# dominikh/jello

Hardware: AMD Instinct MI355X
Metric: Mpixels/sec fine-raster + paths/sec, 100k-path 4096^2 scene (higher is better)
Workload: dtype f32

## Files before the change

jello_amd/csrc/kernels_flatten.hip:

```cpp
#include <hip/hip_runtime.h>
__shared__ double fl_atan_tab[9];
#define JD_ATAN_TAB_LDS fl_atan_tab
#include "kcommon.h"
#define FF_INLINE __device__ __forceinline__
#include "flatten_fast.h"

using namespace jk;
using namespace jd;

namespace {

struct CubicParams { float th0, th1, chord_len, err; };
struct EulerParams { float th0, th1, k0, k1, ch; };
struct CubicPoints { V2 p0, p1, p2, p3; };
struct PointDeriv { V2 point, deriv; };
struct PathTagData { uint32_t tag_byte; MonoidK<5> monoid; };

#define DERIV_THRESH 1e-6f
#define DERIV_THRESH_SQUARED (DERIV_THRESH * DERIV_THRESH)
#define DERIV_EPS 1e-6f
#define SUBDIV_LIMIT (1.0f / 65536.0f)
#define K1_THRESH 1e-3f
#define DIST_THRESH 1e-3f
#define TANGENT_THRESH 1e-6f
// ... 777 lines not shown
        bool is_stroke_cap_marker = (g.tag.tag_byte & JL_PATH_TAG_SUBPATH_END) != 0u;
        if (is_stroke_cap_marker) {
            V2 tangent = cubic_start_tangent(pts.p0, pts.p1, pts.p2, pts.p3);
            V2 offset_tangent = offset * normalize(tangent);
            V2 n = v2(offset_tangent.y * -1.0f, offset_tangent.x * 1.0f);
            draw_cap<EMIT>(o, path_ix, (style_flags & JL_STYLE_FLAGS_START_CAP_MASK) >> 2, pts.p0, pts.p0 - n, pts.p0 + n, -offset_tangent,
                           transform);
        } else {
            const float TT = TANGENT_THRESH * TANGENT_THRESH;
            V2 tan_prev = cubic_end_tangent(pts.p0, pts.p1, pts.p2, pts.p3);
            if (dot(tan_prev, tan_prev) < TT) tan_prev = v2(TANGENT_THRESH, 0.0f);
            V2 offset_tangent = offset * normalize(tan_prev);
            V2 n_prev = v2(offset_tangent.y * -1.0f, offset_tangent.x * 1.0f);
            if (sub < 2u) {
                V2 tan_start = cubic_start_tangent(pts.p0, pts.p1, pts.p2, pts.p3);
                if (dot(tan_start, tan_start) < TT) tan_start = v2(TANGENT_THRESH, 0.0f);
                V2 n_start = offset * normalize(v2(-tan_start.y, tan_start.x));
                job.valid = true; job.cubic = pts; job.local_to_device = transform;
                if (sub == 0u) { job.offset = offset; job.start_p = pts.p0 + n_start; job.end_p = pts.p3 + n_prev; }
                else { job.offset = -offset; job.start_p = pts.p0 - n_start; job.end_p = pts.p3 - n_prev; }
            } else {
                PathTagData ntag = compute_tag_monoid(s, ix + 1u);
                CubicPoints npts = read_path_segment(s, ntag, true);
                bool n_is_closed = (ntag.tag_byte & JL_PATH_TAG_SEG_TYPE) == JL_PATH_TAG_LINETO;
                bool n_is_marker = (ntag.tag_byte & JL_PATH_TAG_SUBPATH_END) != 0u;
                bool do_join = !n_is_marker || n_is_closed;
                if (do_join) {
                    V2 tan_next = cubic_start_tangent(npts.p0, npts.p1, npts.p2, npts.p3);
                    if (dot(tan_next, tan_next) < TT) tan_next = v2(TANGENT_THRESH, 0.0f);
                    V2 tnn = normalize(tan_next);
                    V2 n_next = v2((offset * tnn.y) * -1.0f, (offset * tnn.x) * 1.0f);
                    draw_join<EMIT>(o, path_ix, style_flags, pts.p3, tan_prev, tan_next, n_prev, n_next, transform);
                } else {
                    draw_cap<EMIT>(o, path_ix, (style_flags & JL_STYLE_FLAGS_END_CAP_MASK), pts.p3, pts.p3 + n_prev, pts.p3 - n_prev, offset_tangent,
                                   transform);
                }
            }
        }
    } else {
        job.valid = true; job.cubic = pts; job.local_to_device = transform;
        job.offset = 0.0f; job.start_p = pts.p0; job.end_p = pts.p3;
    }
}

#ifndef FLQ_STACK
#define FLQ_STACK 448u
#endif
#ifndef FLQ_LEAVES
#define FLQ_LEAVES 640u
#endif
#ifndef FLQ_MAX_LEVEL
#define FLQ_MAX_LEVEL 9u
#endif
struct FlBatch {
    uint32_t jhead[64];
    uint32_t stack[FLQ_STACK];
    uint32_t l_tpos[FLQ_LEAVES];
    uint16_t l_key[FLQ_LEAVES];
    uint16_t l_link[FLQ_LEAVES];
    uint32_t unsure[128];
    uint32_t n_stack, n_leaves, bail, n_unsure;
};
JD float lanef(float v, uint32_t src) { return u2f((uint32_t)__builtin_amdgcn_ds_bpermute((int)(src << 2), (int)f2u(v))); }
JD uint32_t laneu(uint32_t v, uint32_t src) { return (uint32_t)__builtin_amdgcn_ds_bpermute((int)(src << 2), (int)v); }

struct NodeResult {
    bool accept;
    CubicParams cp;
    V2 es_p0, es_p1;
    bool ends_at_one;
};
struct NodeEnds {
    V2 last_p, last_q;
    float last_t;
    V2 point, deriv;
    float t1;
};
JD NodeEnds node_ends(V2 p0, V2 p1, V2 p2, V2 p3, uint32_t level, uint32_t t0_u) {
    const float dt = u2f((127u - level) << 23);
    const float t0 = (float)t0_u * dt;
    NodeEnds r;
    if (t0_u == 0u) {
        r.last_p = p0;
        r.last_q = p1 - p0;
        if (dot(r.last_q, r.last_q) < DERIV_THRESH_SQUARED) r.last_q = eval_cubic_and_deriv(p0, p1, p2, p3, DERIV_EPS).deriv;
        r.last_t = 0.0f;
    } else {
        PointDeriv pq0 = eval_cubic_and_deriv(p0, p1, p2, p3, t0);
        r.last_t = t0;
        if (dot(pq0.deriv, pq0.deriv) < DERIV_THRESH_SQUARED) {
            PointDeriv n0 = eval_cubic_and_deriv(p0, p1, p2, p3, t0 - DERIV_EPS);
            pq0.deriv = n0.deriv;
            pq0.point = n0.point;
            r.last_t = t0 - DERIV_EPS;
        }
        r.last_p = pq0.point;
        r.last_q = pq0.deriv;
    }
    float t1 = t0 + dt;
    PointDeriv this_pq1 = eval_cubic_and_deriv(p0, p1, p2, p3, t1);
    if (dot(this_pq1.deriv, this_pq1.deriv) < DERIV_THRESH_SQUARED) {
        PointDeriv new_pq1 = eval_cubic_and_deriv(p0, p1, p2, p3, t1 - DERIV_EPS);
        this_pq1.deriv = new_pq1.deriv;
        if (t1 < 1.0f) {
            this_pq1.point = new_pq1.point;
            t1 = t1 - DERIV_EPS;
        }
    }
    r.point = this_pq1.point;
    r.deriv = this_pq1.deriv;
    r.t1 = t1;
    return r;
}
JD NodeResult node_test(V2 p0, V2 p1, V2 p2, V2 p3, float scale, uint32_t level, uint32_t t0_u) {
    const float tol = 0.25f;
    const float dt = u2f((127u - level) << 23);
    const NodeEnds ne = node_ends(p0, p1, p2, p3, level, t0_u);
    const float actual_dt = ne.t1 - ne.last_t;
    NodeResult r;
    r.cp = cubic_from_points_derivs(ne.last_p, ne.point, ne.last_q, ne.deriv, actual_dt);
    r.accept = r.cp.err * scale <= tol || dt <= SUBDIV_LIMIT;
    r.es_p0 = ne.last_p;
    r.es_p1 = ne.point;
    r.ends_at_one = ne.t1 == 1.0f;
    return r;
}
JD int node_test_fast(V2 p0, V2 p1, V2 p2, V2 p3, float scale, uint32_t level, uint32_t t0_u, float* v_est, float* delta) {
    const float tol = 0.25f;
    const NodeEnds ne = node_ends(p0, p1, p2, p3, level, t0_u);
    const float actual_dt = ne.t1 - ne.last_t;
    const V2 chord = ne.point - ne.last_p;
    const float chord_squared = dot(chord, chord);
    const V2 q0 = ne.last_q, q1 = ne.deriv;
    *v_est = 0.0f; *delta = 0.0f;
    if (chord_squared < DERIV_THRESH_SQUARED) {
        const float chord_err = sqrt_((float)(9.0 / 32.0) * (dot(q0, q0) + dot(q1, q1))) * actual_dt;
        return (chord_err * scale <= tol) ? ffast::FF_ACCEPT : ffast::FF_REJECT;
    }
    const float chord_len = FF_SQRT(chord_squared);
    const float sc = actual_dt * FF_RCP(chord_squared);
    const V2 h0 = v2(q0.x * chord.x + q0.y * chord.y, q0.y * chord.x - q0.x * chord.y);
    const V2 h1 = v2(q1.x * chord.x + q1.y * chord.y, q1.x * chord.y - q1.y * chord.x);
    const float len0 = FF_SQRT(h0.x * h0.x + h0.y * h0.y), len1 = FF_SQRT(h1.x * h1.x + h1.y * h1.y);
    return ffast::ff_decide(h0.x, h0.y, len0, h1.x, h1.y, len1, len0 * sc, len1 * sc, chord_len, scale, tol, v_est, delta);
}
JD CubicParams piece_angles(const NodeEnds& ne) {
    const V2 chord = ne.point - ne.last_p;
    const float chord_squared = dot(chord, chord);
    CubicParams r;
    r.err = 0.0f;
    if (chord_squared < DERIV_THRESH_SQUARED) {
        r.th0 = 0.0f; r.th1 = 0.0f; r.chord_len = DERIV_THRESH;
        return r;
    }
    const V2 q0 = ne.last_q, q1 = ne.deriv;
    const V2 h0 = v2(q0.x * chord.x + q0.y * chord.y, q0.y * chord.x - q0.x * chord.y);
    const V2 h1 = v2(q1.x * chord.x + q1.y * chord.y, q1.x * chord.y - q1.y * chord.x);
    r.th0 = atan2_(h0.y, h0.x);
    r.th1 = atan2_(h1.y, h1.x);
    r.chord_len = sqrt_(chord_squared);
    return r;
}

struct PieceParams {
    EulerParams ep;
    float n, noff, int0, integral;
    uint32_t n_u, robust;
};
JD PieceParams piece_params(const CubicParams& cp, float scale, float offset) {
    const float tol = 0.25f;
    PieceParams r;
    r.ep = es_params_from_angles(cp.th0, cp.th1);
    const EulerParams& ep = r.ep;
    float k0 = ep.k0 - 0.5f * ep.k1;
    float k1 = ep.k1;
    float normalized_offset = offset / cp.chord_len;
    float dist_scaled = normalized_offset * ep.ch;
    float scale_multiplier = sqrt_(0.125f * scale * cp.chord_len / (ep.ch * tol));
    float a = 0.0f, b = 0.0f, integral = 0.0f, int0 = 0.0f, n_frac;
    uint32_t robust = 0u;
    if (abs_(k1) < K1_THRESH) {
        float k = ep.k0;
        n_frac = sqrt_(abs_(k * (k * dist_scaled + 1.0f)));
        robust = 1u;
    } else if (abs_(dist_scaled) < DIST_THRESH) {
        a = k1;
        b = k0;
        int0 = pow_1_5_signed(b);
        float int1 = pow_1_5_signed(a + b);
        integral = int1 - int0;
        n_frac = (float)(2.0 / 3.0) * integral / a;
        robust = 2u;
    } else {
        a = -2.0f * dist_scaled * k1;
        b = -1.0f - 2.0f * dist_scaled * k0;
        int0 = espc_int_approx(b);
        float int1 = espc_int_approx(a + b);
        integral = int1 - int0;
        float k_peak = k0 - k1 * b / a;
        float integrand_peak = sqrt_(abs_(k_peak * (k_peak * dist_scaled + 1.0f)));
        n_frac = integral * integrand_peak / a;
    }
    r.n = clamp_(ceil_(n_frac * scale_multiplier), 1.0f, 100.0f);
    r.n_u = to_u32(r.n);
    r.noff = normalized_offset;
    r.int0 = int0;
    r.integral = integral;
    r.robust = robust;
    return r;
}

#ifdef FL_FAST_CHECK
__device__ uint32_t g_ff_stats[8];
#endif
#ifndef FL_WAVES_PER_EU
#define FL_WAVES_PER_EU 4
#endif
#ifndef FL_BLOCKS_PER_CU
#define FL_BLOCKS_PER_CU 4
#endif
#ifdef FL_TIMING
#define FL_TL_WAVES 8192u
#define FL_TL_BATCHES 15u
#define FL_TL_WORDS (2u + 3u * FL_TL_BATCHES)
__device__ unsigned long long g_fl_timeline[FL_TL_WAVES * FL_TL_WORDS];
#endif
__global__ __launch_bounds__(JL_WG) __attribute__((amdgpu_waves_per_eu(FL_WAVES_PER_EU, FL_WAVES_PER_EU))) void k_flatten_items(const JlConfig* __restrict__ cfg, Buf<uint32_t> scene, Buf<JlTagMonoid> tag_monoids,
                                                         Buf<JlPathBbox> path_bboxes, const uint32_t* __restrict__ list,
                                                         uint32_t* __restrict__ counters, uint32_t cap, uint32_t* __restrict__ counts,
                                                         FlTemp T, uint32_t debug) {
    __shared__ FlBatch sh_batch[JL_WG / 64];
    Scene s;
    s.cfg = cfg; s.scene = scene; s.tag_monoids = tag_monoids;
    uint32_t n_heavy = umin_(counters[0], cap), n_light = umin_(counters[FL_CTR_LIGHT], cap - n_heavy);
    uint32_t n = n_heavy + n_light;
    const uint32_t units_h = n_heavy / 64u + (n_heavy % 64u != 0u ? 1u : 0u);
    const uint32_t units = units_h + n_light / 64u + (n_light % 64u != 0u ? 1u : 0u);
    const uint32_t n_groups = umin_(umax_(gridDim.x / FL_BLOCKS_PER_CU, 1u), FL_DEAL_GROUPS), group = blockIdx.x % n_groups;
    if (group >= units) return;
#ifdef FL_TIMING
    const unsigned long long tl_entry = wall_clock64();
    const uint32_t tl_wave = blockIdx.x * (JL_WG / 64u) + (threadIdx.x >> 6);
    uint32_t tl_n = 0u;
#endif
    atan_tab_fill();
    __syncthreads();
    const uint32_t lane = lane_id();
    FlBatch& B = sh_batch[threadIdx.x >> 6];
    Out<true> o;
    o.cfg = cfg; o.T = T; o.home_s = o.home_r = blockIdx.x % T.K; o.failed_s = o.failed_r = false; o.slot = 0u;
    if ((debug & 1u) != 0u) o.home_s = o.home_r = 0u;
#ifdef FL_SOAK_HOME0
    o.home_s = o.home_r = 0u;
#endif
    o.cursor = 0u; o.a_first = 0u; o.a_spos = 0u; o.a_rpos = 0u;
    for (;;) {
        uint32_t k = 0u;
        if (lane == 0u) k = atomicAdd(&counters[FL_CTR_DEAL + FL_DEAL_STRIDE * group], 1u);
        k = (uint32_t)__builtin_amdgcn_readfirstlane((int)k);
        const uint32_t u = k * n_groups + group;
        if (u >= units) break;
        const bool heavy = u < units_h;
        const uint32_t t_first = heavy ? u * 64u : n_heavy + (u - units_h) * 64u;
        const uint32_t t_end = umin_(t_first + 64u, heavy ? n_heavy : n);
        const uint32_t t = t_first + lane;
#ifdef FL_TIMING
        const unsigned long long tl_start = wall_clock64() | (heavy ? 1ull << 63 : 0ull);
        uint32_t tl_info = 0u;
#define FL_TL_END()                                                                                      \
    do {                                                                                                 \
        if (lane == 0u && tl_wave < FL_TL_WAVES && tl_n < FL_TL_BATCHES) {                               \
            g_fl_timeline[tl_wave * FL_TL_WORDS + 2u + 3u * tl_n] = tl_start;                            \
            g_fl_timeline[tl_wave * FL_TL_WORDS + 3u + 3u * tl_n] = wall_clock64();                      \
            g_fl_timeline[tl_wave * FL_TL_WORDS + 4u + 3u * tl_n] = tl_info;                             \
        }                                                                                                \
        tl_n++;                                                                                          \
    } while (0)
#else
#define FL_TL_END() do {} while (0)
#endif
        if (__builtin_amdgcn_ballot_w64(o.failed_s) != 0ull) { o.home_s = fl_next_home(T, o.home_s, 0); o.failed_s = false; }
        if (__builtin_amdgcn_ballot_w64(o.failed_r) != 0ull) { o.home_r = fl_next_home(T, o.home_r, 1); o.failed_r = false; }
        EulerJob job;
        job.valid = false; job.path_ix = 0u; job.trans_ix = 0u; job.offset = 0.0f;
        job.start_p = v2(0, 0); job.end_p = v2(0, 0);
        job.cubic.p0 = job.cubic.p1 = job.cubic.p2 = job.cubic.p3 = v2(0, 0);
        job.local_to_device = xf_identity();
        uint32_t slot = FL_INVALID;
        if (t < t_end) {
            slot = heavy ? list[t] : list[cap - 1u - (t - n_heavy)];
            o.slot = slot; o.cursor = 0u; o.a_first = 0u; o.a_spos = 0u; o.a_rpos = 0u;
            uint32_t path_ix;
            run_item<true>(cfg, s, o, slot, job, path_ix);
            if (!job.valid) counts[slot] = o.cursor;
        }
        EulerLane e;
        euler_begin(e, job);
        const bool active = job.valid && !e.done;
        if (__builtin_amdgcn_ballot_w64(active) == 0ull) {
            FL_TL_END();
            continue;
        }
        B.jhead[lane] = 0u;
        {
            const uint64_t am = __builtin_amdgcn_ballot_w64(active);
            if (active) B.stack[(uint32_t)__builtin_popcountll(am & ((1ull << lane) - 1ull))] = lane;
            if (lane == 0u) { B.n_stack = (uint32_t)__builtin_popcountll(am); B.n_leaves = 0u; B.bail = 0u; B.n_unsure = 0u; }
        }
        wave_fence();
#ifdef FL_SPLIT_NO_A
        if (lane == 0u) B.n_stack = 0u;
        wave_fence();
#endif
        for (;;) {
#ifdef FL_TIMING
            tl_info += 1u << 16;
#endif
            const uint32_t ns = (uint32_t)__builtin_amdgcn_readfirstlane((int)B.n_stack);
            const uint32_t nu = (uint32_t)__builtin_amdgcn_readfirstlane((int)B.n_unsure);
            if (ns == 0u && nu == 0u) break;
            const bool exact_round = ns == 0u || nu >= 64u;
            const uint32_t take = umin_(exact_round ? nu : ns, 64u);
            const bool has = lane < take;
            const uint32_t node = has ? (exact_round ? B.unsure[nu - 1u - lane] : B.stack[ns - 1u - lane]) : 0u;
            wave_fence();
            const uint32_t j = node & 63u, level = (node >> 6) & 31u, t0_u = node >> 11;
            const V2 jp0 = v2(lanef(e.p0.x, j), lanef(e.p0.y, j)), jp1 = v2(lanef(e.p1.x, j), lanef(e.p1.y, j));
            const V2 jp2 = v2(lanef(e.p2.x, j), lanef(e.p2.y, j)), jp3 = v2(lanef(e.p3.x, j), lanef(e.p3.y, j));
            const float scale = lanef(e.scale, j);
            int kind = ffast::FF_UNSURE;
            if (exact_round) {
                if (has) kind = node_test(jp0, jp1, jp2, jp3, scale, level, t0_u).accept ? ffast::FF_ACCEPT : ffast::FF_REJECT;
            } else if (has) {
                float v_est, delta;
                kind = node_test_fast(jp0, jp1, jp2, jp3, scale, level, t0_u, &v_est, &delta);
#ifdef FL_FAST_CHECK
            }
            if (!exact_round) {
                bool c_unsure = false, c_contra = false, c_viol = false;
                if (has) {
                    float v2_, d2_;
                    const int k2 = node_test_fast(jp0, jp1, jp2, jp3, scale, level, t0_u, &v2_, &d2_);
                    const NodeResult rx = node_test(jp0, jp1, jp2, jp3, scale, level, t0_u);
                    const float vx = rx.cp.err * scale;
                    c_unsure = k2 == ffast::FF_UNSURE;
                    c_contra = (k2 == ffast::FF_ACCEPT && !rx.accept) || (k2 == ffast::FF_REJECT && rx.accept);
                    c_viol = (d2_ > 0.0f && !(abs_(v2_ - vx) <= d2_)) || (d2_ == 0.0f && k2 != ffast::FF_UNSURE && v2_ != 0.0f);
                }
                const uint32_t n0 = (uint32_t)__builtin_popcountll(__builtin_amdgcn_ballot_w64(has));
                const uint32_t n1 = (uint32_t)__builtin_popcountll(__builtin_amdgcn_ballot_w64(c_unsure));
                const uint32_t n2 = (uint32_t)__builtin_popcountll(__builtin_amdgcn_ballot_w64(c_contra));
                const uint32_t n3 = (uint32_t)__builtin_popcountll(__builtin_amdgcn_ballot_w64(c_viol));
                if (lane == 0u) {
                    atomicAdd(&g_ff_stats[0], n0);
                    if (n1) atomicAdd(&g_ff_stats[1], n1);
                    if (n2) atomicAdd(&g_ff_stats[2], n2);
                    if (n3) atomicAdd(&g_ff_stats[3], n3);
                }
#endif
            }
            const bool acc = has && kind == ffast::FF_ACCEPT, rej = has && kind == ffast::FF_REJECT, uns = has && kind == ffast::FF_UNSURE;
            const uint64_t accm = __builtin_amdgcn_ballot_w64(acc), rejm = __builtin_amdgcn_ballot_w64(rej), unsm = __builtin_amdgcn_ballot_w64(uns);
            const uint32_t n_acc = (uint32_t)__builtin_popcountll(accm), n_rej = (uint32_t)__builtin_popcountll(rejm);
            const uint32_t n_uns = (uint32_t)__builtin_popcountll(unsm);
            const uint32_t nl = (uint32_t)__builtin_amdgcn_readfirstlane((int)B.n_leaves);
            const uint32_t ns_left = exact_round ? ns : ns - take, nu_left = exact_round ? nu - take : nu;
            const bool too_deep = __builtin_amdgcn_ballot_w64(rej && level + 1u > FLQ_MAX_LEVEL) != 0ull;
            if (too_deep || ns_left + 2u * n_rej > FLQ_STACK || nl + n_acc > FLQ_LEAVES) {
                if (lane == 0u) B.bail = 1u;
                wave_fence();
                break;
            }
            const uint64_t below = (1ull << lane) - 1ull;
            if (rej) {
                const uint32_t pos = ns_left + 2u * (uint32_t)__builtin_popcountll(rejm & below);
                B.stack[pos] = j | ((level + 1u) << 6) | ((2u * t0_u + 1u) << 11);
                B.stack[pos + 1u] = j | ((level + 1u) << 6) | ((2u * t0_u) << 11);
            }
            if (acc) {
                const uint32_t li = nl + (uint32_t)__builtin_popcountll(accm & below);
                B.l_tpos[li] = node;
                B.l_key[li] = (uint16_t)((t0_u << (FLQ_MAX_LEVEL - level)) << 7);
                const uint32_t prev = atomicExch(&B.jhead[j], li + 1u);
                B.l_link[li] = (uint16_t)((j << 10) | prev);
            }
            if (uns) B.unsure[nu_left + (uint32_t)__builtin_popcountll(unsm & below)] = node;
            if (lane == 0u) { B.n_stack = ns_left + 2u * n_rej; B.n_leaves = nl + n_acc; B.n_unsure = nu_left + n_uns; }
            wave_fence();
        }
        const bool bail = (uint32_t)__builtin_amdgcn_readfirstlane((int)B.bail) != 0u;
        const uint32_t nl = bail ? 0u : (uint32_t)__builtin_amdgcn_readfirstlane((int)B.n_leaves);
#ifdef FL_TIMING
        tl_info = (tl_info & 0x7fff0000u) | (nl & 0xffffu) | (bail ? 1u << 31 : 0u);
#endif
        uint32_t rec_base = 0u;
        if (nl != 0u && lane == 0u) rec_base = fl_grab<1>(T, o.home_r, nl, o.failed_r);
        rec_base = (uint32_t)__builtin_amdgcn_readlane((int)rec_base, 0);
#ifdef FL_SPLIT_NO_B
        for (uint32_t lbase = nl; lbase < nl; lbase += 64u) {
#else
        for (uint32_t lbase = 0u; lbase < nl; lbase += 64u) {
#endif
            const uint32_t li = lbase + lane;
            const bool has = li < nl;
            const uint32_t node = has ? B.l_tpos[li] : 0u;
            const uint32_t j = node & 63u, level = (node >> 6) & 31u, t0_u = node >> 11;
            const V2 jp0 = v2(lanef(e.p0.x, j), lanef(e.p0.y, j)), jp1 = v2(lanef(e.p1.x, j), lanef(e.p1.y, j));
            const V2 jp2 = v2(lanef(e.p2.x, j), lanef(e.p2.y, j)), jp3 = v2(lanef(e.p3.x, j), lanef(e.p3.y, j));
            const float scale = lanef(e.scale, j), offset = lanef(e.offset, j);
            const uint32_t j_slot = laneu(slot, j), j_path = laneu(e.path_ix, j), j_trans = laneu(e.trans_ix, j);
            const float j_tsx = lanef(e.t_start.x, j), j_tsy = lanef(e.t_start.y, j), j_tex = lanef(e.t_end.x, j), j_tey = lanef(e.t_end.y, j);
            if (has) {
                const NodeEnds ne = node_ends(jp0, jp1, jp2, jp3, level, t0_u);
                const CubicParams cp = piece_angles(ne);
                const PieceParams pp = piece_params(cp, scale, offset);
                const uint32_t fl = pp.robust | ((ne.t1 == 1.0f) ? 4u : 0u) | ((offset >= 0.0f) ? 8u : 0u) | ((offset == 0.0f) ? 16u : 0u) |
                                    ((t0_u == 0u) ? 32u : 0u);
                const uint32_t r = rec_base + li;
                if (rec_base != FL_INVALID)
                    piece_record_write(T.recs + (size_t)r * 4u, ne.last_p, ne.point, pp.ep.th0, pp.ep.th1, pp.int0, pp.integral, pp.noff, j_slot, j_path,
                                       j_trans, fl, 0u, v2(j_tsx, j_tsy), v2(j_tex, j_tey));
                B.l_key[li] = (uint16_t)(B.l_key[li] | pp.n_u);
            }
        }
        wave_fence();
        if (nl != 0u) {
            uint32_t total = 0u;
            if (active)
                for (uint32_t q = B.jhead[lane]; q != 0u; q = B.l_link[q - 1u] & 1023u) total += B.l_key[q - 1u] & 127u;
            if (active) counts[slot] = total;
            const uint32_t incl = wave_incl_scan_u32(total);
            const uint32_t batch_total = (uint32_t)__builtin_amdgcn_readlane((int)incl, 63);
            const bool together = batch_total <= ((debug & 4u) != 0u ? 48u : FL_MAX_GRAB);
            uint32_t grab = 0u;
            if (together) {
                if (lane == 0u) grab = fl_grab<0>(T, o.home_s, batch_total, o.failed_s);
            } else if (active && total != 0u) {
                grab = fl_grab<0>(T, o.home_s, total, o.failed_s);
            }
            for (uint32_t li = lane; li < nl; li += 64u) {
                const uint32_t j = B.l_link[li] >> 10, key = B.l_key[li];
                uint32_t first = 0u;
                for (uint32_t q = B.jhead[j]; q != 0u; q = B.l_link[q - 1u] & 1023u) {
                    const uint32_t k2 = B.l_key[q - 1u];
                    if ((k2 >> 7) < (key >> 7)) first += k2 & 127u;
                }
                B.l_tpos[li] = first;
            }
            {
                const uint32_t base0 = (uint32_t)__builtin_amdgcn_readlane((int)grab, 0);
                B.unsure[lane] = together ? (base0 == FL_INVALID ? FL_INVALID : base0 + (incl - total)) : grab;
            }
            wave_fence();
            for (uint32_t li = lane; li < nl; li += 64u) {
                const uint32_t j = B.l_link[li] >> 10, key = B.l_key[li], first = B.l_tpos[li];
                const uint32_t r = rec_base + li, jb = B.unsure[j];
                if (rec_base != FL_INVALID && (key >> 7) != 0u) ((uint32_t*)T.recs)[(size_t)r * 16u + 12u] = first;
                if (jb == FL_INVALID) continue;
                if (rec_base != FL_INVALID) piece_slots_write(T.sinfo, jb + first, key & 127u, r);
                else for (uint32_t i = 0u; i < (key & 127u); i++) T.sinfo[jb + first + i] = make_uint2(0u, 0u);
            }
            wave_fence();
        }
        if (__builtin_expect(bail, 0)) {
            o.slot = slot; o.cursor = 0u; o.a_first = 0u; o.a_spos = 0u; o.a_rpos = 0u;
            bool have = active;
            auto finish = [&]() -> bool {
                if (e.done && have) {
                    counts[o.slot] = o.cursor;
                    have = false;
                }
                return __builtin_amdgcn_ballot_w64(!e.done) != 0ull;
            };
            flatten_euler_wave(o, e, finish);
        }
        FL_TL_END();
    }
#ifdef FL_TIMING
    if (lane == 0u && tl_wave < FL_TL_WAVES) {
        g_fl_timeline[tl_wave * FL_TL_WORDS] = tl_entry;
        g_fl_timeline[tl_wave * FL_TL_WORDS + 1u] = tl_n;
    }
#endif
#undef FL_TL_END
}

#ifndef FL_LINES_WAVES_PER_EU
#define FL_LINES_WAVES_PER_EU 4
#endif
__global__ __launch_bounds__(JL_WG) __attribute__((amdgpu_waves_per_eu(FL_LINES_WAVES_PER_EU, FL_LINES_WAVES_PER_EU))) void k_flatten_lines(const JlConfig* __restrict__ cfg, Buf<uint32_t> scene, const uint32_t* __restrict__ counters,
                                                         FlTemp T, const uint32_t* __restrict__ bases, uint32_t n_slots, Buf<JlLineSoup> lines) {
    atan_tab_fill();
    const uint32_t lines_lim = umin_(cfg->lines_size, lines.n);
    const uint2* __restrict__ sinfo = T.sinfo;
    const uint4* __restrict__ recs = T.recs;
    const uint32_t n_r = T.K * T.R;
    uint32_t ru[FL_MAX_REGIONS], used[FL_MAX_REGIONS];
    uint32_t units = 0u;
#pragma unroll
    for (uint32_t c = 0u; c < FL_MAX_REGIONS; c++) {
        ru[c] = units;
        used[c] = c < T.K ? umin_(counters[FL_CTR_CURSOR + FL_CUR_STRIDE * c], T.R) : 0u;
        units += (used[c] + JL_WG - 1u) / JL_WG;
    }
    auto fetch_info = [&](uint32_t u) -> uint2 {
        if (u >= units) return make_uint2(0u, 0u);
        uint32_t c = 0u, first_unit = 0u, in_use = used[0];
#pragma unroll
        for (uint32_t q = 1u; q < FL_MAX_REGIONS; q++)
            if (u >= ru[q] && used[q] != 0u) { c = q; first_unit = ru[q]; in_use = used[q]; }
        const uint32_t in_region = (u - first_unit) * JL_WG + threadIdx.x;
        return in_region < in_use ? sinfo[(size_t)c * T.R + in_region] : make_uint2(0u, 0u);
    };
    auto state_of = [&](uint2 si) -> uint32_t {
        if (si.x >= n_r) return 0u;
        return (si.y & FL_INFO_PIECE) != 0u ? 2u : ((si.y & FL_INFO_DIRECT) != 0u ? 1u : 0u);
    };
    auto fetch_rec = [&](uint32_t state, uint32_t r, uint4& r0, uint4& r1, uint4& r2, uint4& r3) {
        r0 = r1 = r2 = r3 = make_uint4(0u, 0u, 0u, 0u);
        const uint4* rec = recs + (size_t)r * 4u;
        if (state != 0u) { r0 = rec[0]; r1 = rec[1]; }
        if (state == 2u) { r2 = rec[2]; r3 = rec[3]; }
    };
    const uint32_t G = gridDim.x;
    uint2 si_a = fetch_info(blockIdx.x), si_b = fetch_info(blockIdx.x + G);
    uint32_t st_a = state_of(si_a);
    uint4 a0, a1, a2, a3;
    fetch_rec(st_a, si_a.x, a0, a1, a2, a3);
    for (uint32_t u = blockIdx.x; u < units; u += G) {
        const uint32_t st = st_a;
        const uint2 si = si_a;
        const uint4 r0 = a0, r1 = a1, r2 = a2, r3 = a3;
        si_a = si_b;
        st_a = state_of(si_a);
        fetch_rec(st_a, si_a.x, a0, a1, a2, a3);
        si_b = fetch_info(u + 2u * G);
        uint32_t widx[3] = {0xffffffffu, 0xffffffffu, 0xffffffffu};
        uint2 wdat[3] = {make_uint2(0u, 0u), make_uint2(0u, 0u), make_uint2(0u, 0u)};
        if (st == 1u) {
            const uint32_t item = r0.x, k = r0.y;
            if (item < n_slots) {
                const uint32_t dst = bases[item] + k;
                if (dst < lines_lim) {
                    widx[0] = dst * 3u; wdat[0] = make_uint2(r0.z, 0u);
                    widx[1] = dst * 3u + 1u; wdat[1] = make_uint2(r1.x, r1.y);
                    widx[2] = dst * 3u + 2u; wdat[2] = make_uint2(r1.z, r1.w);
                }
            }
        } else if (st == 2u) {
            const uint32_t n_u = (si.y >> 8) & 127u, i = si.y & 127u;
            const uint32_t flags = r2.w & 63u;
            const bool last_of_item = i + 1u == n_u && (flags & 4u) != 0u;
            const uint32_t slot = r2.y, k = ((flags & 32u) != 0u ? 0u : r3.x) + i;
            Xf tr;
            if ((flags & 16u) != 0u) {
                tr = xf_identity();
            } else {
                uint32_t tb = cfg->layout.transform_base + (r2.w >> 6) * 6u;
                tr.m0 = u2f(scene.rd(tb)); tr.m1 = u2f(scene.rd(tb + 1u)); tr.m2 = u2f(scene.rd(tb + 2u));
                tr.m3 = u2f(scene.rd(tb + 3u)); tr.t0 = u2f(scene.rd(tb + 4u)); tr.t1 = u2f(scene.rd(tb + 5u));
            }
            const uint32_t slot_base = slot < n_slots ? bases[slot] : 0u;
            V2 lp1;
            if (last_of_item) {
                lp1 = v2(u2f(r3.z), u2f(r3.w));
#if defined(FL_LSPLIT) && FL_LSPLIT == 1
            } else if (true) {
                lp1 = v2(u2f(r0.x) + (float)i, u2f(r0.w) + u2f(r1.x) + u2f(r1.y) + u2f(r1.z) + u2f(r1.w) + u2f(r2.x));
#endif
            } else {
                const EulerParams ep = es_params_from_angles(u2f(r1.x), u2f(r1.y));
                const float noff = u2f(r2.x), n = (float)n_u;
                const float tt = (float)(i + 1u) / n;
                float sarg = tt;
                const uint32_t robust = flags & 3u;
                if (robust != 1u) {
                    const float k0 = ep.k0 - 0.5f * ep.k1, k1 = ep.k1;
                    const float dist_scaled = noff * ep.ch;
                    const float int0 = u2f(r1.z), integral = u2f(r1.w);
                    float a, b;
                    if (robust == 2u) {
                        a = k1;
                        b = k0;
                    } else {
                        a = -2.0f * dist_scaled * k1;
                        b = -1.0f - 2.0f * dist_scaled * k0;
                    }
                    float uu = integral * tt + int0;
                    float inv;
                    if (robust == 2u) inv = pow23_abs_(uu) * sign_(uu); else inv = espc_int_inv_approx(uu);
                    sarg = (inv - b) / a;
                }
                lp1 = es_seg_eval_with_offset(v2(u2f(r0.x), u2f(r0.y)), v2(u2f(r0.z), u2f(r0.w)), ep, sarg, noff);
            }
            const V2 q = xf_apply(tr, lp1);
            if (slot < n_slots) {
                const uint32_t dst = slot_base + k;
                const bool fwd = (flags & 8u) != 0u;
                const bool has_next = !last_of_item && dst + 1u < lines_lim;
                const uint2 hdr = make_uint2(r2.z, 0u), pt = make_uint2(f2u(q.x), f2u(q.y));
                if (dst < lines_lim) {
                    if (k == 0u) {
                        uint2* w = (uint2*)lines.p;
                        const V2 qs = xf_apply(tr, v2(u2f(r3.x), u2f(r3.y)));
                        w[(size_t)dst * 3u] = hdr;
                        w[(size_t)dst * 3u + (fwd ? 1u : 2u)] = make_uint2(f2u(qs.x), f2u(qs.y));
                    }
                    widx[0] = dst * 3u + (fwd ? 2u : 1u); wdat[0] = pt;
                    if (has_next) {
                        widx[1] = dst * 3u + 3u; wdat[1] = hdr;
                        widx[2] = dst * 3u + (fwd ? 4u : 5u); wdat[2] = pt;
                    }
                }
            }
        }
        {
            uint2* w = (uint2*)lines.p;
#pragma unroll
            for (int j = 0; j < 3; j++)
#if defined(FL_LSPLIT) && FL_LSPLIT == 2
                if (widx[j] == 0xfffffffeu) w[widx[j]] = wdat[j];
#else
                if (widx[j] != 0xffffffffu) w[widx[j]] = wdat[j];
#endif
        }
    }
}

JD uint32_t fkey(float f) { uint32_t b = f2u(f); return (b & 0x80000000u) ? ~b : (b | 0x80000000u); }
JD float fkey_inv(uint32_t k) { return u2f((k & 0x80000000u) ? (k & 0x7fffffffu) : ~k); }

JD bool fb_tag_has_extent(const uint32_t* __restrict__ bases, uint32_t n_tags, const JlLineSoup* lines, uint32_t total, uint32_t pos) {
    uint32_t g = 0u, ge = n_tags;
    while (ge - g > 1u) {
        const uint32_t mid = g + (ge - g) / 2u;
        if (umin_(bases[3u * mid], total) <= pos) g = mid; else ge = mid;
    }
    const uint32_t lo = umin_(bases[3u * g], total);
    const uint32_t hi = (g + 1u < n_tags) ? umin_(bases[3u * g + 3u], total) : total;
    float bx0 = 1e31f, by0 = 1e31f, bx1 = -1e31f, by1 = -1e31f;
    for (uint32_t i = lo; i < hi; i++) {
        const JlLineSoup l = lines[i];
        bx0 = fmin_(bx0, fmin_(l.p0[0], l.p1[0])); by0 = fmin_(by0, fmin_(l.p0[1], l.p1[1]));
        bx1 = fmax_(bx1, fmax_(l.p0[0], l.p1[0])); by1 = fmax_(by1, fmax_(l.p0[1], l.p1[1]));
    }
    return bx1 > bx0 || by1 > by0;
}

JD void fb_merge(Buf<JlPathBbox> path_bboxes, uint32_t path_ix, int32_t x0, int32_t y0, int32_t x1, int32_t y1, bool atomic) {
    if (!path_bboxes.ok(path_ix)) return;
    if (x0 == 0x7fffffff && y0 == 0x7fffffff && x1 == (int32_t)0x80000000 && y1 == (int32_t)0x80000000) return;
    JlPathBbox* out = &path_bboxes.p[path_ix];
    if (!atomic) {
        out->x0 = imin_(out->x0, x0); out->y0 = imin_(out->y0, y0);
        out->x1 = imax_(out->x1, x1); out->y1 = imax_(out->y1, y1);
    } else {
        const int32_t cx0 = __hip_atomic_load(&out->x0, __ATOMIC_RELAXED, __HIP_MEMORY_SCOPE_AGENT);
        const int32_t cy0 = __hip_atomic_load(&out->y0, __ATOMIC_RELAXED, __HIP_MEMORY_SCOPE_AGENT);
        const int32_t cx1 = __hip_atomic_load(&out->x1, __ATOMIC_RELAXED, __HIP_MEMORY_SCOPE_AGENT);
        const int32_t cy1 = __hip_atomic_load(&out->y1, __ATOMIC_RELAXED, __HIP_MEMORY_SCOPE_AGENT);
        if (x0 < cx0) atomicMin(&out->x0, x0);
        if (y0 < cy0) atomicMin(&out->y0, y0);
        if (x1 > cx1) atomicMax(&out->x1, x1);
        if (y1 > cy1) atomicMax(&out->y1, y1);
    }
}

#define FB_NONE 0xffffffffu
#ifndef FB_TARGET_WAVES
#define FB_TARGET_WAVES 2048u
#endif
__global__ __launch_bounds__(JL_WG) void k_flatten_bbox(const JlConfig* __restrict__ cfg, const JlBump* __restrict__ bump,
                                                        const uint32_t* __restrict__ bases, uint32_t n_slots, Buf<JlLineSoup> lines,
                                                        Buf<JlPathBbox> path_bboxes, uint32_t* __restrict__ zero, uint32_t zero_n) {
    for (uint32_t i = blockIdx.x * JL_WG + threadIdx.x; i < zero_n; i += gridDim.x * JL_WG) zero[i] = 0u;
    const uint32_t n_tags = n_slots / 3u;
    const uint32_t total = umin_(umin_(bump->lines, cfg->lines_size), lines.n);
    const uint32_t lane = lane_id();
    const uint32_t n_waves = (gridDim.x * JL_WG) >> 6;
    const uint32_t batches = umin_(umax_(((total + 63u) / 64u) / FB_TARGET_WAVES, 1u), 8u);
    for (uint64_t start64 = (uint64_t)((blockIdx.x * JL_WG + threadIdx.x) >> 6) * batches * 64u; start64 < total;
         start64 += (uint64_t)n_waves * batches * 64u) {
        const uint32_t start = (uint32_t)start64;
        const uint32_t end = (uint32_t)(start64 + (uint64_t)batches * 64u < total ? start64 + (uint64_t)batches * 64u : total);
        uint32_t p_before = FB_NONE;
        if (start > 0u) p_before = lines.p[start - 1u].path_ix;
        bool skip_before = false;
// ... 185 lines not shown
```

Measured before the change: 21430.

## Dedupe identical adjacent curves and speculatively evaluate child nodes in idle lanes

```diff
diff --git a/jello_amd/csrc/kernels_flatten.hip b/jello_amd/csrc/kernels_flatten.hip
--- a/jello_amd/csrc/kernels_flatten.hip
+++ b/jello_amd/csrc/kernels_flatten.hip
@@ -1103,10 +1103,19 @@
             continue;
         }
         B.jhead[lane] = 0u;
+        uint64_t followers;
         {
             const uint64_t am = __builtin_amdgcn_ballot_w64(active);
-            if (active) B.stack[(uint32_t)__builtin_popcountll(am & ((1ull << lane) - 1ull))] = lane;
-            if (lane == 0u) { B.n_stack = (uint32_t)__builtin_popcountll(am); B.n_leaves = 0u; B.bail = 0u; B.n_unsure = 0u; }
+#define FL_DIFF_BELOW(v) ((uint32_t)__builtin_amdgcn_update_dpp(0, (int)f2u(v), 0x138, 0xf, 0xf, false) ^ f2u(v))
+            const uint32_t diff = FL_DIFF_BELOW(e.p0.x) | FL_DIFF_BELOW(e.p0.y) | FL_DIFF_BELOW(e.p1.x) | FL_DIFF_BELOW(e.p1.y) | FL_DIFF_BELOW(e.p2.x) |
+                                  FL_DIFF_BELOW(e.p2.y) | FL_DIFF_BELOW(e.p3.x) | FL_DIFF_BELOW(e.p3.y) | FL_DIFF_BELOW(e.scale);
+#undef FL_DIFF_BELOW
+            const bool both = lane != 0u && ((am >> ((lane - 1u) & 63u)) & 3ull) == 3ull;
+            const bool follower = both && diff == 0u && (debug & 16u) == 0u;
+            followers = __builtin_amdgcn_ballot_w64(follower);
+            const uint64_t lead = am & ~followers;
+            if (active && !follower) B.stack[(uint32_t)__builtin_popcountll(lead & ((1ull << lane) - 1ull))] = lane;
+            if (lane == 0u) { B.n_stack = (uint32_t)__builtin_popcountll(lead); B.n_leaves = 0u; B.bail = 0u; B.n_unsure = 0u; }
         }
         wave_fence();
 #ifdef FL_SPLIT_NO_A
@@ -1122,9 +1131,12 @@
             if (ns == 0u && nu == 0u) break;
             const bool exact_round = ns == 0u || nu >= 64u;
             const uint32_t take = umin_(exact_round ? nu : ns, 64u);
-            const bool has = lane < take;
-            const uint32_t node = has ? (exact_round ? B.unsure[nu - 1u - lane] : B.stack[ns - 1u - lane]) : 0u;
+            const uint32_t n_ahead = (exact_round || (debug & 32u) != 0u) ? 0u : umin_(take, (64u - take) >> 1);
+            const bool has = lane < take + 2u * n_ahead, half = lane >= take;
+            const uint32_t src = half ? (lane - take) >> 1 : lane;
+            uint32_t node = has ? (exact_round ? B.unsure[nu - 1u - src] : B.stack[ns - 1u - src]) : 0u;
             wave_fence();
+            if (half) node = (node & 63u) | ((((node >> 6) & 31u) + 1u) << 6) | ((2u * (node >> 11) + ((lane - take) & 1u)) << 11);
             const uint32_t j = node & 63u, level = (node >> 6) & 31u, t0_u = node >> 11;
             const V2 jp0 = v2(lanef(e.p0.x, j), lanef(e.p0.y, j)), jp1 = v2(lanef(e.p1.x, j), lanef(e.p1.y, j));
             const V2 jp2 = v2(lanef(e.p2.x, j), lanef(e.p2.y, j)), jp3 = v2(lanef(e.p3.x, j), lanef(e.p3.y, j));
@@ -1160,13 +1172,22 @@
                 }
 #endif
             }
-            const bool acc = has && kind == ffast::FF_ACCEPT, rej = has && kind == ffast::FF_REJECT, uns = has && kind == ffast::FF_UNSURE;
-            const uint64_t accm = __builtin_amdgcn_ballot_w64(acc), rejm = __builtin_amdgcn_ballot_w64(rej), unsm = __builtin_amdgcn_ballot_w64(uns);
-            const uint32_t n_acc = (uint32_t)__builtin_popcountll(accm), n_rej = (uint32_t)__builtin_popcountll(rejm);
-            const uint32_t n_uns = (uint32_t)__builtin_popcountll(unsm);
+            const uint64_t rej0 = __builtin_amdgcn_ballot_w64(has && !half && kind == ffast::FF_REJECT);
+            const bool live = has && (!half || ((rej0 >> src) & 1ull) != 0ull);
+            const bool acc = live && kind == ffast::FF_ACCEPT, rej_any = live && kind == ffast::FF_REJECT, uns = live && kind == ffast::FF_UNSURE;
+            const bool rej = rej_any && (half || lane >= n_ahead);
+            const uint64_t rejm = __builtin_amdgcn_ballot_w64(rej), unsm = __builtin_amdgcn_ballot_w64(uns);
+            const uint32_t n_rej = (uint32_t)__builtin_popcountll(rejm), n_uns = (uint32_t)__builtin_popcountll(unsm);
+            const uint32_t n_mem = acc ? 1u + (j == 63u ? 0u : (uint32_t)__builtin_ctzll(~(followers >> (j + 1u)))) : 0u;
+            uint32_t n_acc = 0u;
+            for (uint32_t m = 0u;; m++) {
+                const uint64_t mm = __builtin_amdgcn_ballot_w64(m < n_mem);
+                if (mm == 0ull) break;
+                n_acc += (uint32_t)__builtin_popcountll(mm);
+            }
             const uint32_t nl = (uint32_t)__builtin_amdgcn_readfirstlane((int)B.n_leaves);
             const uint32_t ns_left = exact_round ? ns : ns - take, nu_left = exact_round ? nu - take : nu;
-            const bool too_deep = __builtin_amdgcn_ballot_w64(rej && level + 1u > FLQ_MAX_LEVEL) != 0ull;
+            const bool too_deep = __builtin_amdgcn_ballot_w64(rej_any && level + 1u > FLQ_MAX_LEVEL) != 0ull;
             if (too_deep || ns_left + 2u * n_rej > FLQ_STACK || nl + n_acc > FLQ_LEAVES) {
                 if (lane == 0u) B.bail = 1u;
                 wave_fence();
@@ -1178,12 +1199,22 @@
                 B.stack[pos] = j | ((level + 1u) << 6) | ((2u * t0_u + 1u) << 11);
                 B.stack[pos + 1u] = j | ((level + 1u) << 6) | ((2u * t0_u) << 11);
             }
-            if (acc) {
-                const uint32_t li = nl + (uint32_t)__builtin_popcountll(accm & below);
-                B.l_tpos[li] = node;
-                B.l_key[li] = (uint16_t)((t0_u << (FLQ_MAX_LEVEL - level)) << 7);
-                const uint32_t prev = atomicExch(&B.jhead[j], li + 1u);
-                B.l_link[li] = (uint16_t)((j << 10) | prev);
+            {
+                const uint16_t key = (uint16_t)((t0_u << ((FLQ_MAX_LEVEL - level) & 15u)) << 7);
+                uint32_t li0 = nl;
+                for (uint32_t m = 0u;; m++) {
+                    const bool mine = m < n_mem;
+                    const uint64_t mm = __builtin_amdgcn_ballot_w64(mine);
+                    if (mm == 0ull) break;
+                    if (mine) {
+                        const uint32_t li = li0 + (uint32_t)__builtin_popcountll(mm & below), jm = j + m;
+                        B.l_tpos[li] = (node & ~63u) | jm;
+                        B.l_key[li] = key;
+                        const uint32_t prev = atomicExch(&B.jhead[jm], li + 1u);
+                        B.l_link[li] = (uint16_t)((jm << 10) | prev);
+                    }
+                    li0 += (uint32_t)__builtin_popcountll(mm);
+                }
             }
             if (uns) B.unsure[nu_left + (uint32_t)__builtin_popcountll(unsm & below)] = node;
             if (lane == 0u) { B.n_stack = ns_left + 2u * n_rej; B.n_leaves = nl + n_acc; B.n_unsure = nu_left + n_uns; }
```

Result: no change. 21600 (median of 6 runs) (+0.8%).
